# Jan-Celin/SCCG-genome-compression

Measured on AMD Instinct MI355X. Metric: target bases compressed/sec at 1/2/4/8 GPUs; bit-exact record stream vs CPU ref, higher is better.
Workload: dtype u8

## Files before the change

### sccg-genome-compression_amd/csrc/walk.hip

```cpp
#include "internal.h"

#include <algorithm>
#include <chrono>
#include <map>
#include <mutex>
#include <cstdio>
#include <cstdlib>
#include <vector>

namespace {

constexpr int WPB = 4;
constexpr int WWPB = 4;
constexpr int WCAP = 256;
constexpr int32_t INVALID = INT32_MIN;
constexpr int32_t NEVER = INT32_MIN + 1;
constexpr int ANCHOR_K = 32;
constexpr int KEY_K = 15;
constexpr int KMAX = 32;
constexpr int KB_COUNT = 32;
constexpr int ANCHOR_STEP = 64;
constexpr int ANCHOR_LOAD = 1;
constexpr int ANCHOR_PROBE_BATCHES = 2;
constexpr uint32_t A_MULTI = 0xFFFFFFFFu;
// ... 1404 lines not shown
        int32_t e = x0, pe = P0;
        if (i > 0) { e = A.chm_t[i - 1] + A.chm_l[i - 1]; pe = A.chm_p[i - 1] + A.chm_l[i - 1] - 1; }
        sx = e > vc ? e : vc;
        sp = pe;
    };
    int32_t ux, up, i1, ex, ep, i2;
    state_at(lo, lo_c, ux, up, i1);
    state_at(hi, hi_c, ex, ep, i2);
    const int32_t n = i2 - i1;
    const int32_t b = A.cur[q];
    int32_t* ot = A.bt[b] + (size_t)q * A.cap;
    int32_t* op = A.bp[b] + (size_t)q * A.cap;
    int32_t* ol = A.bl[b] + (size_t)q * A.cap;
    for (int32_t i = lane; i < n; i += 64) { ot[i] = A.chm_t[i1 + i]; op[i] = A.chm_p[i1 + i]; ol[i] = A.chm_l[i1 + i]; }
    if (lane == 0) {
        A.cnt[b][q] = n;
        A.usedX[q] = ux; A.usedP[q] = up;
        A.exitX[q] = ex; A.exitP[q] = ep;
        A.changed[q] = 0; A.seedq[q] = 0; A.trapped[q] = 0; A.frozen[q] = 0;
    }
}

__device__ __forceinline__ uint64_t mix64(uint64_t x) {
    x ^= x >> 33; x *= 0xff51afd7ed558ccdull; x ^= x >> 33; x *= 0xc4ceb9fe1a85ec53ull; x ^= x >> 33;
    return x;
}
template <bool ALIGNED>
__device__ __forceinline__ bool code32(const uint8_t* s, uint64_t& code) {
    uint32_t w[8];
    if (ALIGNED) {
        const uint4* p = reinterpret_cast<const uint4*>(s);
        const uint4 a = p[0], b = p[1];
        w[0] = a.x; w[1] = a.y; w[2] = a.z; w[3] = a.w; w[4] = b.x; w[5] = b.y; w[6] = b.z; w[7] = b.w;
    } else {
        loadw<8>(s, w);
    }
    uint32_t bad;
    pack_codes<8>(w, code, bad);
    return bad == 0;
}

constexpr uint32_t ANCHOR_GEN_MASK = 0xfffu;
__device__ __forceinline__ uint64_t anchor_slot(const WalkPtrs& A, uint64_t key, uint32_t pos) {
    return ((uint64_t)(A.agen & ANCHOR_GEN_MASK) << 52) | ((uint64_t)(uint32_t)(key & 0xfffffu) << 32) | pos;
}
__device__ __forceinline__ bool anchor_hit(const WalkPtrs& A, uint64_t key, uint64_t v) {
    return (v >> 32) == (anchor_slot(A, key, 0) >> 32) && (uint32_t)v != A_MULTI;
}
__device__ __forceinline__ void anchor_put(const WalkPtrs& A, uint64_t key, uint32_t pos) {
    if (A.adet) atomicMax((unsigned long long*)&A.atab[key >> (64 - A.abits)], (unsigned long long)anchor_slot(A, key, pos));
    else A.atab[key >> (64 - A.abits)] = anchor_slot(A, key, pos);
}

__device__ __forceinline__ void anchor_samples(const WalkPtrs& A, int64_t nR, int64_t p0, const uint32_t (&cw)[20],
                                               const uint32_t (&dw)[20], uint32_t acc) {
    const int nh = A.astep == 32 ? 2 : 1;
#pragma unroll
    for (int h = 0; h < 2; h++) {
        const int64_t p = p0 + 32 * h;
        if (h >= nh || p + ANCHOR_K > nR) break;
        uint64_t code = 0;
        uint32_t bad = 0;
#pragma unroll
        for (int i = 0; i < 8; i++) {
            code |= (uint64_t)cw[8 * h + i] << (8 * i);
            bad |= dw[8 * h + i];
        }
        if (acc && bad) continue;
        const uint64_t key = mix64(code);
        anchor_put(A, key, (uint32_t)p);
    }
}

__device__ __forceinline__ int32_t anchor_diag_f(int32_t nT, const uint8_t* __restrict__ T, const uint64_t* __restrict__ atab, int32_t abits,
                                 uint32_t agen, int32_t y0) {
    const int lane = lane_id();
    constexpr int NB = ANCHOR_PROBE_BATCHES;
    const uint64_t tag = ((uint64_t)(agen & ANCHOR_GEN_MASK) << 52);
    int32_t dg[NB];
#pragma unroll
    for (int b = 0; b < NB; b++) {
        const int32_t y = y0 + b * 64 + lane;
        dg[b] = INVALID;
        uint64_t code;
        if (y + ANCHOR_K <= nT && code32<false>(T + y, code)) {
            const uint64_t key = mix64(code);
            const uint64_t v = atab[key >> (64 - abits)];
            if ((v >> 32) == ((tag | ((uint64_t)(uint32_t)(key & 0xfffffu) << 32)) >> 32) && (uint32_t)v != A_MULTI)
                dg[b] = (int32_t)(uint32_t)v - y;
        }
    }
    int32_t g = INVALID, first = INVALID;
    int gv = 1;
    for (int tries = 0; tries < 8; tries++) {
        int32_t d = INVALID;
#pragma unroll
        for (int b = 0; b < NB; b++) {
            const unsigned long long m = __ballot(dg[b] != INVALID);
            if (m && d == INVALID) d = __shfl(dg[b], first_lane(m), 64);
        }
        if (d == INVALID) break;
        if (first == INVALID) first = d;
        int votes = 0;
#pragma unroll
        for (int b = 0; b < NB; b++) {
            votes += __popcll(__ballot(dg[b] == d));
            if (dg[b] == d) dg[b] = INVALID;
        }
        if (votes > gv) { g = d; gv = votes; }
    }
    return g == INVALID ? first : g;
}
__device__ int32_t anchor_diag(const WalkPtrs& A, int32_t y0) { return anchor_diag_f(A.nT, A.T, A.atab, A.abits, A.agen, y0); }


constexpr int FC_PER_T = 64;

__device__ __forceinline__ int32_t serial_ext(const uint8_t* R, int32_t nR, const uint8_t* T, int32_t nT, int32_t c,
                                              int32_t y, int k) {
    int32_t l = k;
    while (c + l < nR && y + l < nT && R[c + l] == T[y + l]) ++l;
    return l;
}

template <typename Pred, typename Hit, typename Words>
__device__ __forceinline__ void sweep_kmers_w(const uint8_t* __restrict__ R, int64_t npos, int k, Pred&& pred, Hit&& hit,
                                              Words&& words);
template <typename Pred, typename Hit>
__device__ __forceinline__ void sweep_kmers(const uint8_t* __restrict__ R, int64_t npos, int k, Pred&& pred, Hit&& hit) {
    sweep_kmers_w(R, npos, k, pred, hit, [](int64_t, const uint32_t (&)[20], const uint32_t (&)[20], uint32_t) {});
}
template <typename Pred, typename Hit, typename Words>
__device__ __forceinline__ void sweep_kmers_w(const uint8_t* __restrict__ R, int64_t npos, int k, Pred&& pred, Hit&& hit,
                                              Words&& words) {
    const uint32_t MASK = (1u << (2 * k)) - 1u, KM = (1u << k) - 1u;
    const int64_t stride = (int64_t)gridDim.x * blockDim.x * FC_PER_T;
    for (int64_t p0 = ((int64_t)blockIdx.x * blockDim.x + threadIdx.x) * FC_PER_T; p0 < npos; p0 += stride) {
        uint32_t cw[20], dw[20], acc = 0;
        {
            const uint4* src = reinterpret_cast<const uint4*>(R + p0);
            uint32_t w[20];
#pragma unroll
            for (int i = 0; i < 5; i++) {
                const uint4 v = src[i];
                w[4 * i] = v.x; w[4 * i + 1] = v.y; w[4 * i + 2] = v.z; w[4 * i + 3] = v.w;
            }
#pragma unroll
            for (int i = 0; i < 20; i++) { cw[i] = swar_codes(w[i], dw[i]); acc |= dw[i]; }
        }
        words(p0, cw, dw, acc);
        uint64_t hits = 0;
#pragma unroll
        for (int g = 0; g < 4; g++) {
            uint64_t code = 0;
            uint32_t bad = 0;
#pragma unroll
            for (int i = 0; i < 8; i++) code |= (uint64_t)cw[4 * g + i] << (8 * i);
            if (acc) {
                const uint4* gp = reinterpret_cast<const uint4*>(R + p0 + 16 * g);
                const uint4 v0 = gp[0], v1 = gp[1];
                const uint32_t gw[8] = {v0.x, v0.y, v0.z, v0.w, v1.x, v1.y, v1.z, v1.w};
#pragma unroll
                for (int i = 0; i < 8; i++) { uint32_t d; swar_codes(gw[i], d); bad |= nz_bytes(d) << (4 * i); }
            }
            uint32_t m16 = 0;
            if (!acc) {
#pragma unroll
                for (int st = 15; st >= 0; st--) m16 = (m16 << 1) | (uint32_t)pred((uint32_t)(code >> (2 * st)) & MASK, true);
            } else {
#pragma unroll
                for (int st = 15; st >= 0; st--)
                    m16 = (m16 << 1) | (uint32_t)pred((uint32_t)(code >> (2 * st)) & MASK, ((bad >> st) & KM) == 0);
            }
            hits |= (uint64_t)m16 << (16 * g);
        }
        if (p0 + FC_PER_T > npos) hits &= npos - p0 >= 64 ? ~0ull : ((1ull << (npos - p0)) - 1);
        while (hits) {
            const int b = __ffsll((long long)hits) - 1;
            hits &= hits - 1;
            hit(p0 + b);
        }
    }
}

__global__ void k_fullc(WalkPtrs A, int32_t y, int32_t P, int pass) {
    const int k = A.k, kp = A.kp;
    const uint8_t* kb = A.T + y;
    const uint32_t key = walk_key(kb, kp);
    const uint32_t lmax = (uint32_t)A.fc[0];
    const bool exo = key >= KEY_EXOTIC;
    sweep_kmers(A.R, (int64_t)A.nR - k + 1, kp, [&](uint32_t code, bool pure) {
        return exo ? !pure : (pure && code == key);
    }, [&](int64_t c) {
        if ((exo || k > kp) && !bytes_eq(A.R + c, kb, k)) return;
        const int32_t l = serial_ext(A.R, A.nR, A.T, A.nT, (int32_t)c, y, k);
        if (pass == 0) atomicMax(&A.fc[0], (unsigned long long)l);
        else if ((uint32_t)l == lmax) {
            atomicAdd(&A.fc[1], 1ull);
            if (c == 0) atomicOr(&A.fc[2], 1ull);
            else atomicMin(&A.fc[3], (unsigned long long)pick_key((int32_t)c, P));
        }
    });
}

constexpr int PB = 1024;
constexpr int PBBITS = 11;
constexpr int PRESENCE_GRID = 1024;
constexpr unsigned KEY0_GRID = 1024;
constexpr int KEY0_GRID_MAX = 16384;
constexpr int PFBITS = 17;

struct CandBest {
    uint32_t l, cnt, has0;
    uint64_t minkey;
};
__device__ __forceinline__ CandBest cb_merge(const CandBest& a, const CandBest& b) {
    if (a.l > b.l) return a;
    if (b.l > a.l) return b;
    return CandBest{a.l, a.cnt + b.cnt, a.has0 | b.has0, a.minkey < b.minkey ? a.minkey : b.minkey};
}
__device__ __forceinline__ CandBest cb_shfl_xor(const CandBest& v, int d) {
    return CandBest{(uint32_t)__shfl_xor((int)v.l, d, 64), (uint32_t)__shfl_xor((int)v.cnt, d, 64),
                    (uint32_t)__shfl_xor((int)v.has0, d, 64), (uint64_t)__shfl_xor((unsigned long long)v.minkey, d, 64)};
}
__device__ __forceinline__ CandBest cb_wave(CandBest v) {
#pragma unroll
    for (int d = 32; d > 0; d >>= 1) v = cb_merge(v, cb_shfl_xor(v, d));
    return v;
}

__global__ __launch_bounds__(SCCG_BLOCK) void k_presence(WalkPtrs A, int32_t x0, int32_t nb) {
    __shared__ uint32_t hkey[1 << PBBITS];
    __shared__ uint32_t hidx[1 << PBBITS];
    __shared__ uint32_t bits[1 << (PFBITS - 5)];
    __shared__ CandBest wbest[SCCG_BLOCK / 64];
    const int k = A.k, kp = A.kp;
    const uint32_t key0 = walk_key(A.T + x0, kp);
    CandBest best{0, 0, 0, ~0ull};
    for (int i = threadIdx.x; i < (1 << PBBITS); i += blockDim.x) { hkey[i] = 0xffffffffu; hidx[i] = 0xffffffffu; }
    for (int i = threadIdx.x; i < (1 << (PFBITS - 5)); i += blockDim.x) bits[i] = 0;
    __syncthreads();
    for (int i = threadIdx.x; i < nb; i += blockDim.x) {
        uint32_t w[4], bad;
        uint64_t cw;
        loadw<4>(A.T + x0 + i, w);
        pack_codes<4>(w, cw, bad);
        const uint32_t key = bad & ((1u << kp) - 1u) ? exotic_key(A.T + x0 + i, kp) : (uint32_t)cw & ((1u << (2 * kp)) - 1u);
        if (key >= KEY_EXOTIC) { atomicMin(&A.fc[5], (unsigned long long)(x0 + i)); continue; }
        const uint32_t fb = slot_hash(key, PFBITS);
        atomicOr(&bits[fb >> 5], 1u << (fb & 31));
        int slot = (int)slot_hash(key, PBBITS);
        for (;;) {
            const uint32_t prev = atomicCAS(&hkey[slot], 0xffffffffu, key);
            if (prev == 0xffffffffu || prev == key) { atomicMin(&hidx[slot], (uint32_t)i); break; }
            slot = (slot + 1) & ((1 << PBBITS) - 1);
        }
    }
    __syncthreads();
    sweep_kmers(A.R, (int64_t)A.nR - k + 1, kp, [&](uint32_t code, bool pure) {
        const uint32_t fb = slot_hash(code, PFBITS);
        return pure && ((bits[fb >> 5] >> (fb & 31)) & 1u);
    }, [&](int64_t c) {
        uint64_t cw = 0;
        uint32_t bad;
        uint32_t w[4];
        loadw<4>(A.R + c, w);
        pack_codes<4>(w, cw, bad);
        const uint32_t code = (uint32_t)cw & ((1u << (2 * kp)) - 1u);
        if (code == key0 && (k == kp || bytes_eq(A.R + c + kp, A.T + x0 + kp, k - kp))) {
            const uint32_t l = (uint32_t)serial_ext(A.R, A.nR, A.T, A.nT, (int32_t)c, x0, k);
            best = cb_merge(best, CandBest{l, 1u, c == 0 ? 1u : 0u, c ? pick_key((int32_t)c, -1) : ~0ull});
        }
        int slot = (int)slot_hash(code, PBBITS);
        for (;;) {
            const uint32_t hk = hkey[slot];
            if (hk == 0xffffffffu) break;
            if (hk == code) { atomicMin(&A.fc[4], (unsigned long long)(x0 + hidx[slot])); break; }
            slot = (slot + 1) & ((1 << PBBITS) - 1);
        }
    });
    best = cb_wave(best);
    if (lane_id() == 0) wbest[wave_in_block()] = best;
    __syncthreads();
    if (threadIdx.x == 0) {
        for (int i = 1; i < SCCG_BLOCK / 64; i++) best = cb_merge(best, wbest[i]);
        unsigned long long* o = A.fcb + 4 * blockIdx.x;
        o[0] = best.l; o[1] = best.cnt; o[2] = best.has0; o[3] = best.minkey;
    }
}

template <bool ANCH>
__global__ __launch_bounds__(SCCG_BLOCK) void k_key0(WalkPtrs A, int32_t x0) {
    __shared__ CandBest wbest[SCCG_BLOCK / 64];
    const int k = A.k, kp = A.kp;
    const uint32_t key0 = walk_key(A.T + x0, kp);
    CandBest best{0, 0, 0, ~0ull};
    if (key0 < KEY_EXOTIC || ANCH) {
        const bool want = key0 < KEY_EXOTIC;
        sweep_kmers_w(A.R, (int64_t)A.nR - k + 1, kp, [&](uint32_t code, bool pure) { return want && pure && code == key0; },
                      [&](int64_t c) {
                          if (k > kp && !bytes_eq(A.R + c + kp, A.T + x0 + kp, k - kp)) return;
                          const uint32_t l = (uint32_t)serial_ext(A.R, A.nR, A.T, A.nT, (int32_t)c, x0, k);
                          best = cb_merge(best, CandBest{l, 1u, c == 0 ? 1u : 0u, c ? pick_key((int32_t)c, -1) : ~0ull});
                      },
                      [&](int64_t p0, const uint32_t (&cw)[20], const uint32_t (&dw)[20], uint32_t acc) {
                          if (ANCH) anchor_samples(A, A.nR, p0, cw, dw, acc);
                      });
    }
    best = cb_wave(best);
    if (lane_id() == 0) wbest[wave_in_block()] = best;
    __syncthreads();
    if (threadIdx.x == 0) {
        for (int i = 1; i < SCCG_BLOCK / 64; i++) best = cb_merge(best, wbest[i]);
        unsigned long long* o = A.fcb + 4 * blockIdx.x;
        o[0] = best.l; o[1] = best.cnt; o[2] = best.has0; o[3] = best.minkey;
    }
}

__global__ __launch_bounds__(SCCG_BLOCK) void k_first_kmer(const uint8_t* __restrict__ fa, int64_t n,
                                                           const int64_t* __restrict__ hdr, int k, int64_t limit,
                                                           uint8_t* __restrict__ kb) {
    __shared__ int64_t tmp[5];
    constexpr int PER = 64;
    const int64_t h = hdr[0], he = hdr[1];
    const int64_t end = n < limit ? n : limit;
    int64_t found = 0;
    for (int64_t base = 0; base < end && found < k; base += (int64_t)SCCG_BLOCK * PER) {
        const int64_t p0 = base + (int64_t)threadIdx.x * PER;
        uint32_t w[PER / 4];
        if (p0 + PER + 4 <= end) {
            loadw<PER / 4>(fa + p0, w);
        } else {
#pragma unroll
            for (int q = 0; q < PER / 4; q++) {
                uint32_t v = 0;
                for (int i = 0; i < 4; i++) {
                    const int64_t p = p0 + 4 * q + i;
                    v |= (uint32_t)(p < end ? fa[p] : (uint8_t)' ') << (8 * i);
                }
                w[q] = v;
            }
        }
        uint64_t keep = 0;
#pragma unroll
        for (int i = 0; i < PER; i++) {
            const uint8_t b = (uint8_t)(w[i >> 2] >> (8 * (i & 3)));
            const int64_t p = p0 + i;
            const bool kp = p < end && !(p >= h && p < he) && !c_isspace(b) && c_toupper(b) != 'N';
            keep |= (uint64_t)kp << i;
        }
        int64_t total = 0;
        int64_t idx = found + block_excl_add((int64_t)__popcll(keep), tmp, &total);
        for (uint64_t m = keep; m && idx < k; m &= m - 1, idx++) {
            const int i = __ffsll((long long)m) - 1;
            kb[idx] = c_toupper((uint8_t)(w[i >> 2] >> (8 * (i & 3))));
        }
        found += total;
    }
    if (threadIdx.x == 0) *reinterpret_cast<int32_t*>(kb + KB_COUNT) = found < k ? (int32_t)found : k;
}

__global__ __launch_bounds__(SCCG_BLOCK) void k_sweep_early(WalkPtrs A) {
    const int k = A.k, kp = A.kp;
    const int64_t nR = A.dnR ? *A.dnR : A.nR;
    const bool have = *reinterpret_cast<const int32_t*>(A.kb + KB_COUNT) == k;
    const uint32_t key0 = have ? walk_key(A.kb, kp) : KEY_EXOTIC;
    const bool want = key0 < KEY_EXOTIC;
    sweep_kmers_w(A.R, nR - k + 1, kp, [&](uint32_t code, bool pure) { return want && pure && code == key0; },
                  [&](int64_t c) {
                      if (k > kp && !bytes_eq(A.R + c + kp, A.kb + kp, k - kp)) return;
                      const unsigned long long i = atomicAdd(&A.fc[13], 1ull);
                      if (i < (unsigned long long)CAND_CAP) A.cand[i] = (int32_t)c;
                  },
                  [&](int64_t p0, const uint32_t (&cw)[20], const uint32_t (&dw)[20], uint32_t acc) {
                      anchor_samples(A, nR, p0, cw, dw, acc);
                  });
}

constexpr int CAND_STATS_GRID = 256;
__device__ __forceinline__ bool cand_stats_usable(const WalkPtrs& A) {
    const int k = A.k, lane = lane_id();
    const bool head = *reinterpret_cast<const int32_t*>(A.kb + KB_COUNT) == k && A.fc[13] <= (unsigned long long)CAND_CAP &&
                      A.nT >= k;
    const bool same = lane >= k || A.kb[lane] == A.T[lane];
    return head && __ballot(!same) == 0 && walk_key(A.kb, A.kp) < KEY_EXOTIC;
}
__global__ __launch_bounds__(SCCG_BLOCK) void k_cand_stats(WalkPtrs A) {
    __shared__ CandBest wbest[SCCG_BLOCK / 64];
    __shared__ int ok, last;
    const int k = A.k;
    const unsigned long long cnt = A.fc[13];
    if (threadIdx.x < 64) {
        const bool u = cand_stats_usable(A);
        if (threadIdx.x == 0) ok = u;
    }
    __syncthreads();
    CandBest v{0, 0, 0, ~0ull};
    if (ok) {
        const unsigned long long nw = (unsigned long long)gridDim.x * (SCCG_BLOCK / 64);
        for (unsigned long long i = blockIdx.x * (SCCG_BLOCK / 64) + (threadIdx.x >> 6); i < cnt; i += nw) {
            const int32_t c = A.cand[i];
            int32_t maxlen = A.nR - (c + k);
            if (A.nT - k < maxlen) maxlen = A.nT - k;
            const uint32_t l = (uint32_t)(k + wave_lce_hbm(A.R, c + k, A.T, k, maxlen));
            v = cb_merge(v, CandBest{l, 1u, c == 0 ? 1u : 0u, c ? pick_key(c, -1) : ~0ull});
        }
    }
    if (lane_id() != 0) v = CandBest{0, 0, 0, ~0ull};
    v = cb_wave(v);
    if (lane_id() == 0) wbest[threadIdx.x >> 6] = v;
    __syncthreads();
    if (threadIdx.x == 0) {
        for (int i = 1; i < SCCG_BLOCK / 64; i++) v = cb_merge(v, wbest[i]);
        unsigned long long* o = A.fcb + 4 * blockIdx.x;
        o[0] = v.l; o[1] = v.cnt; o[2] = v.has0; o[3] = v.minkey;
    }
    if (!grid_last_block(reinterpret_cast<unsigned int*>(A.fc + 14), &last)) return;
    if (threadIdx.x == 0) A.fc[12] = ok ? 1 : 2;
    if (!ok) return;
    v = CandBest{0, 0, 0, ~0ull};
    for (int b = (int)threadIdx.x; b < (int)gridDim.x; b += SCCG_BLOCK) {
        const unsigned long long* o = A.fcb + 4 * b;
        v = cb_merge(v, CandBest{(uint32_t)o[0], (uint32_t)o[1], (uint32_t)o[2], o[3]});
    }
    v = cb_wave(v);
    if (lane_id() == 0) wbest[threadIdx.x >> 6] = v;
    __syncthreads();
    if (threadIdx.x == 0) {
// ... 264 lines not shown
        wave_copy(A.T + src, out + dst, len);
    }
}

__global__ __launch_bounds__(SCCG_BLOCK) void k_copy(const uint8_t* __restrict__ in, int64_t n, uint8_t* __restrict__ out) {
    const int64_t G = (int64_t)gridDim.x * WPB;
    for (int64_t o = ((int64_t)blockIdx.x * WPB + wave_in_block()) * LONG_PIECE; o < n; o += G * LONG_PIECE)
        wave_copy(in + o, out + o, n - o < LONG_PIECE ? n - o : LONG_PIECE);
}

struct Carve {
    char* base;
    size_t off, cap;
    template <typename T>
    T* take(size_t n) {
        off = (off + 255) & ~(size_t)255;
        T* p = reinterpret_cast<T*>(base + off);
        off += n * sizeof(T);
        return p;
    }
};

int env_int(const char* name, int dflt) {
    const char* e = getenv(name);
    return e ? atoi(e) : dflt;
}
struct WalkEnv {
    bool debug;
    bool phases;
    int debug_round;
    int debug_rounds;
    bool all_rounds;
    int debug_chunk;
    int round_log;
};
const WalkEnv& walk_env() {
    static const WalkEnv e = [] {
        const char* rl = getenv("SCCG_ROUND_LOG");
        return WalkEnv{getenv("SCCG_DEBUG") != nullptr,       getenv("SCCG_DEBUG_PHASES") != nullptr,
                       env_int("SCCG_DEBUG_ROUND", -1),       env_int("SCCG_DEBUG_ROUNDS", 3),
                       getenv("SCCG_DEBUG_ALLROUNDS") != nullptr, env_int("SCCG_DEBUG_CHUNK", -1),
                       rl ? (rl[0] == '2' ? 2 : 1) : 0};
    }();
    return e;
}

int anchor_bits(int64_t nR) {
    static const int shift = [] { const int x = env_int("SCCG_ANCHOR_SHIFT", 0); return x >= -4 && x <= 4 ? x : 0; }();
    int64_t want = ANCHOR_LOAD * (nR / ANCHOR_STEP + 1);
    int b = 10;
    while ((1ll << b) < want && b < 34) b++;
    b += shift;
    return b < 10 ? 10 : b;
}

WalkPtrs carve(void* ws, size_t ws_bytes, const uint8_t* R, int64_t nR, const uint8_t* T, int64_t nT, int k, int m,
               int S, size_t* used, int abits = 0) {
    WalkPtrs A{};
    Carve c{(char*)ws, 0, ws_bytes};
    A.R = R; A.T = T;
    A.nR = (int32_t)nR; A.nT = (int32_t)nT; A.k = k; A.m = m; A.S = S;
    A.kp = k < KEY_K ? k : KEY_K;
    A.C = (int32_t)((nT + S - 1) / S);
    if (A.C < 1) A.C = 1;
    A.xlo = 0;
    A.xhi = (int32_t)nT;
    A.cap = S / k + 4;
    const size_t C = (size_t)A.C, cap = (size_t)A.cap;
    A.abits = abits ? abits : anchor_bits(nR);
    A.astep = ANCHOR_STEP;
    A.atab = c.take<uint64_t>((size_t)1 << A.abits);
    A.fc = c.take<unsigned long long>(16);
    A.fcb = c.take<unsigned long long>(4 * KEY0_GRID_MAX);
    A.cand = c.take<int32_t>(CAND_CAP);
    A.kb = c.take<uint8_t>(64);
    for (int b = 0; b < 2; b++) {
        A.bt[b] = c.take<int32_t>(C * cap);
        A.bp[b] = c.take<int32_t>(C * cap);
        A.bl[b] = c.take<int32_t>(C * cap);
        A.cnt[b] = c.take<int32_t>(C);
    }
    A.cur = c.take<int32_t>(C);
    A.exitX = c.take<int32_t>(C); A.exitP = c.take<int32_t>(C);
    A.usedX = c.take<int32_t>(C); A.usedP = c.take<int32_t>(C);
    A.kind = c.take<int32_t>(C); A.status = c.take<int32_t>(C);
    A.escX = c.take<int32_t>(C); A.escP = c.take<int32_t>(C); A.escN = c.take<int32_t>(C); A.escQ = c.take<int32_t>(C);
    A.snapX = c.take<int32_t>(C); A.snapP = c.take<int32_t>(C);
    A.guess = c.take<int32_t>(C);
    A.plist = c.take<int32_t>(C);
    A.rlist = c.take<int32_t>(C);
    A.clist = c.take<int32_t>(C);
    A.newX = c.take<int32_t>(C); A.newP = c.take<int32_t>(C);
    A.conv = c.take<int32_t>(C); A.changed = c.take<int32_t>(C); A.walked = c.take<int32_t>(C);
    A.lround = c.take<int32_t>(C);
    A.seedq = c.take<int32_t>(C);
    A.trapped = c.take<int32_t>(C);
    A.frozen = c.take<int32_t>(C); A.flist = c.take<int32_t>(C);
    A.fbits = c.take<uint32_t>(C / 32 + 1); A.cbits = c.take<uint32_t>(C / 32 + 1);
    A.fy = c.take<int32_t>(FROZEN_MAX);
    A.scal = c.take<int32_t>(16);
    A.trig = c.take<int32_t>(RESPEC_MAX_TRIGGERS);
    A.tflag = c.take<int32_t>(C);
    A.fa_j = c.take<int32_t>(FROZEN_MAX); A.fa_l = c.take<int32_t>(FROZEN_MAX); A.fa_p = c.take<int32_t>(FROZEN_MAX);
    A.hintY = c.take<int32_t>(C); A.hintP = c.take<int32_t>(C);
    A.flat_off = c.take<int64_t>(C + 1);
    const size_t maxm = (size_t)(nT / k + 2);
    A.ft = c.take<int32_t>(maxm); A.fp = c.take<int32_t>(maxm); A.fl = c.take<int32_t>(maxm);
    A.tlen = c.take<int64_t>(maxm + 1);
    A.partial = c.take<int64_t>((size_t)scan_partials_needed((int64_t)(maxm > C ? maxm : C) + 1) + 16);
    A.scal64 = c.take<int64_t>(8);
    A.lgap_cap = nT / LONG_GAP + nT / LONG_PIECE + 2;
    A.lgap = c.take<int64_t>(3 * (size_t)A.lgap_cap);
    A.cprev = c.take<int64_t>(C + 1);
    A.ctext = c.take<int64_t>(C + 1);
    A.chs = c.take<int32_t>(16);
    {
        const int64_t mc = nT / k + 2;
        const int64_t lim = CH_HANDBACK_N + 1 < CHAIN_MCAP ? CH_HANDBACK_N + 1 : CHAIN_MCAP;
        A.chm_cap = (int32_t)(mc < lim ? mc : lim);
    }
    A.chm_t = c.take<int32_t>((size_t)A.chm_cap);
    A.chm_p = c.take<int32_t>((size_t)A.chm_cap);
    A.chm_l = c.take<int32_t>((size_t)A.chm_cap);
    A.chh_y = c.take<int32_t>((size_t)CH_GRID * CH_HCAP);
    A.chh_k = c.take<uint32_t>((size_t)CH_GRID * CH_HCAP);
    A.chh_n = c.take<int32_t>(CH_GRID);
    A.chh_tr = c.take<int32_t>(CH_GRID);
    A.dbg = c.take<uint64_t>(C * DBG_SLOTS);
    *used = c.off;
    return A;
}

using WalkKernel = void (*)(WalkPtrs, const int32_t*, int32_t, const int32_t*);
WalkKernel walk_kernel(const WalkPtrs& A) { return A.dbg ? k_walk<true, false> : k_walk<false, false>; }
constexpr int CARRY_GRID = 256;
int launch_carry(const WalkPtrs& A, hipStream_t s) {
    hipLaunchKernelGGL(k_list_sort, dim3(1), dim3(LS_T), 0, s, A, A.clist, (const int32_t*)(A.scal + 11), A.cbits);
    PROF_LAUNCH(PROF_WALK_CARRY, s, (A.dbg ? k_walk<true, true> : k_walk<false, true>), dim3(CARRY_GRID), dim3(64 * WWPB), 0, s, A,
                (const int32_t*)A.clist, 0, (const int32_t*)(A.scal + 11));
    SCCG_HIP(hipGetLastError());
    return 0;
}

struct FullC {
    int64_t lmax;
    int32_t p;
};

int set_u64(unsigned long long* p, std::initializer_list<int64_t> v, hipStream_t s) {
    return dev_set_i64(reinterpret_cast<int64_t*>(p), (int)v.size(), v, s);
}

int run_fullc(WalkPtrs& A, int32_t y, int32_t P, FullC* out, hipStream_t s) {
    int rc = set_u64(A.fc, {0, 0, 0, -1}, s);
    if (rc) return rc;
    const int64_t npos = (int64_t)A.nR - A.k + 1;
    unsigned g = grid_for(npos > 0 ? npos : 1, 256 * FC_PER_T);
    if (g > 8192) g = 8192;
    PROF_LAUNCH(PROF_FULLC, s, k_fullc, dim3(g), dim3(256), 0, s, A, y, P, 0);
    PROF_LAUNCH(PROF_FULLC, s, k_fullc, dim3(g), dim3(256), 0, s, A, y, P, 1);
    SCCG_HIP(hipGetLastError());
    unsigned long long r[4];
    {
        const RbItem it{A.fc, r, (int)sizeof r};
        const int rc = dev_readback(&it, 1, s);
        if (rc) return rc;
    }
    out->lmax = (int64_t)r[0];
    if (r[0] == 0) { out->p = INVALID; return 0; }
    const uint64_t k0 = (uint64_t)(uint32_t)(P < 0 ? -P : P) << 32;
    uint64_t pk;
    if (r[1] >= 2 && r[2]) pk = r[3];
    else pk = (r[2] && k0 < r[3]) ? k0 : r[3];
    out->p = (int32_t)(uint32_t)pk;
    return 0;
}

int h2d_sync(void* dst, const void* src, size_t bytes, hipStream_t s) {
    if (!bytes) return 0;
    SCCG_HIP(hipMemcpyAsync(dst, src, bytes, hipMemcpyHostToDevice, s));
    SCCG_HIP(hipStreamSynchronize(s));
    return 0;
}

int run_chain(WalkPtrs& A, hipStream_t s, int* gens, bool* trapped, bool* started) {
    hipLaunchKernelGGL(k_chain_init, dim3(1), dim3(64), 0, s, A);
    SCCG_HIP(hipGetLastError());
    int32_t st[5] = {0, 0, 0, 0, 0};
    *started = true;
    for (int it = 0;; it++) {
        for (int g = 0; g < CH_GENS_PER_SYNC; g++) {
            hipLaunchKernelGGL(k_chain_scan, dim3(CH_GRID), dim3(1024), 0, s, A);
            hipLaunchKernelGGL(k_chain_step, dim3(1), dim3(64), 0, s, A);
        }
        SCCG_HIP(hipGetLastError());
        const RbItem it0{A.chs, st, (int)sizeof st};
        const int rc = dev_readback(&it0, 1, s);
        if (rc) return rc;
        if (!st[0] && st[4] < 0) {
            *started = false;
            *gens = 0;
            *trapped = false;
            return 0;
        }
        if (!st[0]) break;
        if (it > CH_MAX_GENS / CH_GENS_PER_SYNC + 1) return SCCG_E_INTERNAL;
    }
    PROF_LAUNCH(PROF_WALK_CHAIN, s, k_chain_fill, dim3(grid_for(A.C, WPB)), dim3(SCCG_BLOCK), 0, s, A);
    SCCG_HIP(hipGetLastError());
    int32_t cs[12];
    {
// ... 46 lines not shown
        if (rc) return rc;
        if ((rc = h2d_sync(A.rlist, rl.data(), rl.size() * 4, s))) return rc;
        PROF_LAUNCH(PROF_WALK, s, walk_kernel(A), dim3(grid_for((int64_t)rl.size(), WWPB)), dim3(64 * WWPB), 0, s, A,
                    (const int32_t*)A.rlist, (int32_t)rl.size(), (const int32_t*)nullptr);
        SCCG_HIP(hipGetLastError());
    }
}

}

size_t walk_workspace_bytes(int64_t nR, int64_t nT, int k, int chunk) {
    size_t used = 0;
    carve(nullptr, 0, nullptr, nR, nullptr, nT, k, 100, chunk, &used);
    return used + 4096;
}

static thread_local WalkPtrs g_last;
static thread_local int64_t g_last_n = 0;

int global_matches(void* , const int32_t** t, const int32_t** p, const int32_t** l, int64_t* n) {
    *t = g_last.ft; *p = g_last.fp; *l = g_last.fl; *n = g_last_n;
    return 0;
}

#define RC(expr)                      \
    do {                              \
        int rc_ = (expr);             \
        if (rc_) return rc_;          \
    } while (0)

namespace {

struct Prepared {
    const void* ws = nullptr;
    const uint8_t* R = nullptr;
    const uint8_t* T = nullptr;
    int64_t nR = -1, nT = -1;
    int k = 0, m = 0, chunk = 0;
    uint32_t agen = 0;
    int abits = 0;
};
thread_local Prepared g_prep;

struct Early {
    const void* ws = nullptr;
    const uint8_t* R = nullptr;
    int64_t nR = -1;
    int k = 0;
    uint32_t agen = 0;
    int abits = 0;
};
thread_local Early g_early;

unsigned first_sweep_grid(const WalkPtrs& A) {
    const unsigned g = grid_for(A.nR - A.k + 1, 256 * FC_PER_T);
    return g > KEY0_GRID ? KEY0_GRID : g;
}

struct AnchorSeen { const uint64_t* tab; size_t clean; uint32_t gen; };
std::mutex g_anchor_mu;
std::map<const void*, AnchorSeen> g_anchor_seen;

int anchor_generation(WalkPtrs& A, const void* ws, hipStream_t s) {
    const size_t n = (size_t)1 << A.abits;
    uint32_t g;
    bool clear;
    {
        std::lock_guard<std::mutex> lk(g_anchor_mu);
        AnchorSeen& e = g_anchor_seen[ws];
        clear = e.tab != A.atab || n > e.clean || e.gen >= ANCHOR_GEN_MASK;
        if (clear) e.gen = 0;
        e.tab = A.atab;
        e.clean = n;
        g = ++e.gen;
    }
    if (clear) SCCG_HIP(hipMemsetAsync(A.atab, 0, n * sizeof(uint64_t), s));
    A.agen = g;
    return 0;
}

int queue_prepare(WalkPtrs& A, const void* ws, hipStream_t s) {
    const int32_t lastk = A.nT - A.k;
    const bool walkable = A.nR >= A.k && lastk >= 0;
    if (!walkable) return 0;
    const unsigned gsweep = first_sweep_grid(A);
    RC(anchor_generation(A, ws, s));
    PROF_LAUNCH(PROF_ANCHOR, s, k_key0<true>, dim3(gsweep), dim3(SCCG_BLOCK), 0, s, A, 0);
    hipLaunchKernelGGL(k_cand_reduce, dim3(1), dim3(1024), 0, s, A, (int)gsweep, 0);
    SCCG_HIP(hipGetLastError());
    return 0;
}

WalkPtrs make_ptrs(const uint8_t* Rp, int64_t nRp, const uint8_t* Tp, int64_t nTp, int k, int m, int chunk, void* ws,
                   size_t ws_bytes, size_t* used, int abits = 0) {
    WalkPtrs A = carve(ws, ws_bytes, Rp, nRp, Tp, nTp, k, m, chunk, used, abits);
    if (!walk_env().debug) A.dbg = nullptr;
    A.dbg_phases = walk_env().phases;
    A.dbg_round = walk_env().debug_round;
    A.adet = env_int("SCCG_ANCHOR_DET", 0);
    return A;
}

}

void global_prepare_reset() { g_prep = Prepared{}; g_early = Early{}; }

int global_sweep_early(const uint8_t* Rp, int64_t nRp, const int64_t* d_nRp, const uint8_t* tgt_fa, int64_t tn,
                       const int64_t* d_hdr, int k, int m, int chunk, void* ws, size_t ws_bytes, hipStream_t s_head,
                       hipEvent_t ev_head, hipStream_t s) {
    g_early = Early{};
    if (m < 0 || 2 * m + 1 > WCAP || k > KMAX || k < 1) return SCCG_E_UNSUPPORTED;
    if (nRp < k || tn <= 0) return 0;
    size_t used = 0;
    WalkPtrs A = make_ptrs(Rp, nRp, nullptr, tn, k, m, chunk, ws, ws_bytes, &used);
    if (used > ws_bytes) return SCCG_E_INTERNAL;
    A.dnR = d_nRp;
    RC(anchor_generation(A, ws, s_head));
    RC(set_u64(A.fc + 12, {0, 0, 0}, s_head));
    hipLaunchKernelGGL(k_first_kmer, dim3(1), dim3(SCCG_BLOCK), 0, s_head, tgt_fa, tn, d_hdr, k, (int64_t)1 << 20, A.kb);
    SCCG_HIP(hipEventRecord(ev_head, s_head));
    SCCG_HIP(hipStreamWaitEvent(s, ev_head, 0));
    PROF_LAUNCH(PROF_ANCHOR, s, k_sweep_early, dim3(first_sweep_grid(A)), dim3(SCCG_BLOCK), 0, s, A);
    SCCG_HIP(hipGetLastError());
    g_early = Early{ws, Rp, nRp, k, A.agen, A.abits};
    return 0;
}

int global_prepare(const uint8_t* Rp, int64_t nRp, const uint8_t* Tp, int64_t nTp, int k, int m, int chunk, void* ws,
                   size_t ws_bytes, hipStream_t s) {
    g_prep = Prepared{};
    if (m < 0 || 2 * m + 1 > WCAP || k > KMAX || k < 1) return SCCG_E_UNSUPPORTED;
    const Early e = g_early;
    g_early = Early{};
    const bool early = e.ws == ws && e.R == Rp && e.nR >= nRp && e.k == k;
    size_t used = 0;
    WalkPtrs A = make_ptrs(Rp, nRp, Tp, nTp, k, m, chunk, ws, ws_bytes, &used, early ? e.abits : 0);
    if (used > ws_bytes) return SCCG_E_INTERNAL;
    if (early) {
        A.agen = e.agen;
        if (A.nR >= A.k && A.nT >= A.k) {
            hipLaunchKernelGGL(k_cand_stats, dim3(CAND_STATS_GRID), dim3(SCCG_BLOCK), 0, s, A);
            SCCG_HIP(hipGetLastError());
        }
    } else {
        RC(queue_prepare(A, ws, s));
    }
    g_prep = Prepared{ws, Rp, Tp, nRp, nTp, k, m, chunk, A.agen, A.abits};
    return 0;
}

namespace {
struct RangeWalk {
    int64_t x0 = 0, P0 = -1, x_end = 0;
    int64_t exit_x = 0, exit_P = -1;
};

struct WalkRun {
    WalkPtrs A;
    hipStream_t s;
    WalkResult* res;
    const EmitTarget* late_out;
    RangeWalk* rw;
    uint8_t* out;
    bool abs_p, keep_flat;
    const uint8_t* Tp;
    int64_t nTp;
    int32_t lastk;
    int32_t first_y = INVALID, first_p = 0, first_l = 0;
    int32_t startX = 0, startP = INVALID;
    bool pre_round = false;
    bool spec_queued = false;
    bool spec_text = false;
    bool text_done = false;
    bool resolved = false;
    int32_t rs_pre[6] = {};
// ... 38 lines not shown
    SCCG_HIP(hipGetLastError());
    RC(launch_round_end(A, 0, fbase_cap, s));
    return 0;
}

int WalkRun::queue_text(bool long_copy, bool dev_first) {
    const int32_t nf = dev_first ? 2 : first_y != INVALID ? 1 : 0;
    if (A.C <= CP_MAX) {
        hipLaunchKernelGGL(k_chunk_prefix, dim3(1), dim3(1024), 0, s, A);
    } else {
        const unsigned gc = grid_for(A.C, 256) > 4096 ? 4096 : grid_for(A.C, 256);
        hipLaunchKernelGGL(k_chunk_meta, dim3(gc), dim3(256), 0, s, A);
        RC(dev_excl_max(A.cprev, A.cprev, A.C, nullptr, A.partial, s));
        RC(dev_excl_sum(A.flat_off, A.flat_off, A.C, A.scal64, A.partial, s));
        RC(set_u64(reinterpret_cast<unsigned long long*>(A.scal64 + 2), {0}, s));
    }
    const FirstMatch F{first_y, first_p, first_l, nf};
    hipLaunchKernelGGL(k_chunk_text<false>, dim3(grid_for(A.C, WPB)), dim3(SCCG_BLOCK), 0, s, A, F, (int)abs_p, out);
    RC(dev_excl_sum(A.ctext, A.ctext, A.C, A.scal64 + 1, A.partial, s));
    PROF_LAUNCH(PROF_MATCH_EMIT, s, k_chunk_text<true>, dim3(grid_for(A.C, WPB)), dim3(SCCG_BLOCK), 0, s, A, F,
                (int)abs_p, out);
    if (long_copy) hipLaunchKernelGGL(k_long_copy, dim3(1024), dim3(256), 0, s, A, out);
    SCCG_HIP(hipGetLastError());
    return 0;
}

int WalkRun::frozen_batch(int fbase, int fcap, bool init_fy) {
    if (init_fy) SCCG_HIP(hipMemsetD32Async((hipDeviceptr_t)A.fy, INT32_MAX, fcap, s));
    if (fcap > 0) hipLaunchKernelGGL(k_frozen_scan, dim3(FZ_GRID, fcap), dim3(FZ_T), 0, s, A, fbase);
    SCCG_HIP(hipGetLastError());
    RC(launch_round_end(A, fbase, fcap, s));
    return 0;
}

int WalkRun::first_step() {
    const int k = A.k;
    int32_t x0 = 0;
    unsigned long long r[9];
    if (pre_round) {
        if (!keep_flat && !walk_env().debug) {
            RC(resolve_out());
            RC(queue_text(true, true));
            spec_queued = true;
        }
        const RbItem it[3] = {{A.fc + 4, r, (int)sizeof r}, {A.scal, rs_pre, (int)sizeof rs_pre},
                              {A.scal64, spec_r, (int)sizeof spec_r}};
        RC(dev_readback(it, 3, s));
        if (!(r[8] != 2 && r[0] == 0 && r[4] > 0)) { pre_round = false; spec_queued = false; }
    } else {
        const RbItem it{A.fc + 4, r, (int)sizeof r};
        RC(dev_readback(&it, 1, s));
    }
    if (r[8] == 2) {
        const unsigned g = first_sweep_grid(A);
        hipLaunchKernelGGL(k_key0<false>, dim3(g), dim3(SCCG_BLOCK), 0, s, A, 0);
        hipLaunchKernelGGL(k_cand_reduce, dim3(1), dim3(1024), 0, s, A, (int)g, 0);
        SCCG_HIP(hipGetLastError());
        const RbItem it{A.fc + 4, r, (int)sizeof r};
        RC(dev_readback(&it, 1, s));
    }
    if (r[0] == 0 && r[4] > 0) {
        first_y = 0;
        const uint64_t k0 = 1ull << 32;
        const uint64_t pk = (r[5] >= 2 && r[6]) ? r[7] : ((r[6] && k0 < r[7]) ? k0 : r[7]);
        first_p = (int32_t)(uint32_t)pk;
        first_l = (int32_t)r[4];
    }
    const int64_t npos = (int64_t)A.nR - k + 1 > 0 ? (int64_t)A.nR - k + 1 : 1;
    const unsigned gsweep = grid_for(npos, 256 * FC_PER_T) > PRESENCE_GRID ? PRESENCE_GRID : grid_for(npos, 256 * FC_PER_T);
    while (x0 <= lastk && first_y == INVALID) {
        const int32_t nb = (lastk - x0 + 1) < PB ? (lastk - x0 + 1) : PB;
        RC(set_u64(A.fc + 4, {-1, -1}, s));
        PROF_LAUNCH(PROF_PRESENCE, s, k_presence, dim3(gsweep), dim3(SCCG_BLOCK), 0, s, A, x0, nb);
        hipLaunchKernelGGL(k_cand_reduce, dim3(1), dim3(1024), 0, s, A, (int)gsweep, -1);
        SCCG_HIP(hipGetLastError());
        {
            const RbItem it{A.fc + 4, r, (int)sizeof r};
            RC(dev_readback(&it, 1, s));
        }
        if (r[0] != ~0ull && r[0] < r[1]) {
            const int32_t y = (int32_t)r[0];
            if (y == x0 && r[4] > 0) {
                const uint64_t k0 = 1ull << 32;
                const uint64_t pk = (r[5] >= 2 && r[6]) ? r[7] : ((r[6] && k0 < r[7]) ? k0 : r[7]);
                first_y = y;
                first_p = (int32_t)(uint32_t)pk;
                first_l = (int32_t)r[4];
                break;
            }
            if (A.k == A.kp) { first_y = y; break; }
            FullC f;
            RC(run_fullc(A, y, -1, &f, s));
            if (f.lmax > 0) { first_y = y; first_p = f.p; first_l = (int32_t)f.lmax; break; }
            x0 = y + 1;
            continue;
        }
        if (r[1] != ~0ull) {
            FullC f;
            RC(run_fullc(A, (int32_t)r[1], -1, &f, s));
            if (f.lmax > 0) { first_y = (int32_t)r[1]; break; }
            x0 = (int32_t)r[1] + 1;
            continue;
        }
        x0 += nb;
    }
    if (first_y != INVALID && first_l == 0) {
        FullC f;
        RC(run_fullc(A, first_y, -1, &f, s));
        first_p = f.p;
        first_l = (int32_t)f.lmax;
    }
    return 0;
}

int WalkRun::probe_frozen_first(bool* frozen_first) {
    RC(dev_set_i32(A.flist, 1, {0}, s));
    RC(dev_set_i32(A.exitX, 1, {startX}, s));
    RC(dev_set_i32(A.exitP, 1, {startP}, s));
    RC(dev_set_i32(A.scal + 5, 1, {1}, s));
    RC(dev_set_i32(A.fy, 1, {INT32_MAX}, s));
    hipLaunchKernelGGL(k_frozen_scan, dim3(FZ_GRID, 1), dim3(FZ_T), 0, s, A, 0);
    SCCG_HIP(hipGetLastError());
// ... 450 lines not shown
```

Before: 188.7 billion.

## Restructure k-mer sweep to wave-coalesced tiles with prefetch and key filter

Rewrites the reference k-mer sweep so each wave processes a contiguous span with lane-interleaved 16-byte loads. Neighbour codes come from cross-lane shuffles instead of per-thread 80-byte reloads, and the next tile is software-prefetched. Adds a SWAR prefilter for single-key sweeps that skips per-position predicate evaluation when no match is possible, and a cold path for tiles containing non-ACGT bytes. Grid sizes now derive from occupancy queries instead of fixed caps. This risks more shuffle overhead and register pressure, and adds complexity in the handling of bad bytes at tile boundaries.

```diff
diff --git a/sccg-genome-compression_amd/csrc/walk.hip b/sccg-genome-compression_amd/csrc/walk.hip
--- a/sccg-genome-compression_amd/csrc/walk.hip
+++ b/sccg-genome-compression_amd/csrc/walk.hip
@@ -1480,24 +1480,11 @@
     else A.atab[key >> (64 - A.abits)] = anchor_slot(A, key, pos);
 }
 
-__device__ __forceinline__ void anchor_samples(const WalkPtrs& A, int64_t nR, int64_t p0, const uint32_t (&cw)[20],
-                                               const uint32_t (&dw)[20], uint32_t acc) {
-    const int nh = A.astep == 32 ? 2 : 1;
-#pragma unroll
-    for (int h = 0; h < 2; h++) {
-        const int64_t p = p0 + 32 * h;
-        if (h >= nh || p + ANCHOR_K > nR) break;
-        uint64_t code = 0;
-        uint32_t bad = 0;
-#pragma unroll
-        for (int i = 0; i < 8; i++) {
-            code |= (uint64_t)cw[8 * h + i] << (8 * i);
-            bad |= dw[8 * h + i];
-        }
-        if (acc && bad) continue;
-        const uint64_t key = mix64(code);
-        anchor_put(A, key, (uint32_t)p);
-    }
+__device__ __forceinline__ void anchor_sample(const WalkPtrs& A, int64_t nR, int64_t q, uint32_t mine, uint32_t next,
+                                              uint32_t bad) {
+    if ((q & (int64_t)(A.astep - 1)) != 0 || q + ANCHOR_K > nR || bad) return;
+    const uint64_t key = mix64((uint64_t)mine | ((uint64_t)next << 32));
+    anchor_put(A, key, (uint32_t)q);
 }
 
 __device__ __forceinline__ int32_t anchor_diag_f(int32_t nT, const uint8_t* __restrict__ T, const uint64_t* __restrict__ atab, int32_t abits,
@@ -1542,8 +1529,6 @@
 __device__ int32_t anchor_diag(const WalkPtrs& A, int32_t y0) { return anchor_diag_f(A.nT, A.T, A.atab, A.abits, A.agen, y0); }
 
 
-constexpr int FC_PER_T = 64;
-
 __device__ __forceinline__ int32_t serial_ext(const uint8_t* R, int32_t nR, const uint8_t* T, int32_t nT, int32_t c,
                                               int32_t y, int k) {
     int32_t l = k;
@@ -1551,64 +1536,137 @@
     return l;
 }
 
-template <typename Pred, typename Hit, typename Words>
-__device__ __forceinline__ void sweep_kmers_w(const uint8_t* __restrict__ R, int64_t npos, int k, Pred&& pred, Hit&& hit,
-                                              Words&& words);
-template <typename Pred, typename Hit>
-__device__ __forceinline__ void sweep_kmers(const uint8_t* __restrict__ R, int64_t npos, int k, Pred&& pred, Hit&& hit) {
-    sweep_kmers_w(R, npos, k, pred, hit, [](int64_t, const uint32_t (&)[20], const uint32_t (&)[20], uint32_t) {});
-}
-template <typename Pred, typename Hit, typename Words>
-__device__ __forceinline__ void sweep_kmers_w(const uint8_t* __restrict__ R, int64_t npos, int k, Pred&& pred, Hit&& hit,
-                                              Words&& words) {
+constexpr int SW_PIECES = 4;
+constexpr int SW_SPAN = 64 * 16 * SW_PIECES;
+constexpr int SW_BLOCK_SPAN = (SCCG_BLOCK / 64) * SW_SPAN;
+static_assert(ANCHOR_STEP == 64 && SW_SPAN == 64 * ANCHOR_STEP, "a wave iteration holds one sample per lane");
+
+__device__ __forceinline__ uint32_t sweep_pack(const uint4& v, uint32_t& flag) {
+    const uint32_t xl = __builtin_amdgcn_perm(v.y, v.x, 0x05010400u), xh = __builtin_amdgcn_perm(v.y, v.x, 0x07030602u);
+    const uint32_t zl = __builtin_amdgcn_perm(v.w, v.z, 0x05010400u), zh = __builtin_amdgcn_perm(v.w, v.z, 0x07030602u);
+    const uint32_t u[4] = {__builtin_amdgcn_perm(zl, xl, 0x05040100u), __builtin_amdgcn_perm(zl, xl, 0x07060302u),
+                           __builtin_amdgcn_perm(zh, xh, 0x05040100u), __builtin_amdgcn_perm(zh, xh, 0x07060302u)};
+    uint32_t c[4];
+    flag = 0;
+#pragma unroll
+    for (int i = 0; i < 4; i++) {
+        c[i] = ((u[i] >> 1) ^ (u[i] >> 2)) & 0x03030303u;
+        flag |= __builtin_amdgcn_perm(0x54474341u, 0x54474341u, c[i]) ^ u[i];
+    }
+    return c[0] | (c[1] << 2) | (c[2] << 4) | (c[3] << 6);
+}
+__device__ __forceinline__ uint32_t sweep_bad(const uint4& v) {
+    uint32_t d0, d1, d2, d3;
+    (void)swar_codes(v.x, d0); (void)swar_codes(v.y, d1); (void)swar_codes(v.z, d2); (void)swar_codes(v.w, d3);
+    return nz_bytes(d0) | (nz_bytes(d1) << 4) | (nz_bytes(d2) << 8) | (nz_bytes(d3) << 12);
+}
+
+__device__ __forceinline__ void sweep_load(const uint8_t* __restrict__ R, int64_t nR, int64_t b0, int lane, uint4 (&v)[SW_PIECES + 1]) {
+#pragma unroll
+    for (int j = 0; j <= SW_PIECES; j++) {
+        const int64_t q = b0 + 1024 * j + (j < SW_PIECES ? 16 * lane : 0);
+        v[j] = *reinterpret_cast<const uint4*>(R + (q < nR ? q : 0));
+    }
+}
+
+constexpr int SW_FILTER = 8;
+template <bool SINGLE, typename Pred, typename Hit, typename Words>
+__device__ __forceinline__ void sweep_kmers_w(const uint8_t* __restrict__ R, int64_t nR, int64_t npos, int k, uint32_t key,
+                                              Pred&& pred, Hit&& hit, Words&& words) {
     const uint32_t MASK = (1u << (2 * k)) - 1u, KM = (1u << k) - 1u;
-    const int64_t stride = (int64_t)gridDim.x * blockDim.x * FC_PER_T;
-    for (int64_t p0 = ((int64_t)blockIdx.x * blockDim.x + threadIdx.x) * FC_PER_T; p0 < npos; p0 += stride) {
-        uint32_t cw[20], dw[20], acc = 0;
-        {
-            const uint4* src = reinterpret_cast<const uint4*>(R + p0);
-            uint32_t w[20];
+    const int lane = lane_id();
+    uint32_t kb[SW_FILTER];
 #pragma unroll
-            for (int i = 0; i < 5; i++) {
-                const uint4 v = src[i];
-                w[4 * i] = v.x; w[4 * i + 1] = v.y; w[4 * i + 2] = v.z; w[4 * i + 3] = v.w;
+    for (int i = 0; i < SW_FILTER; i++) kb[i] = 0x55555555u * ((key >> (2 * i)) & 3u);
+    const bool filter = SINGLE && k >= SW_FILTER;
+    const int64_t stride = (int64_t)gridDim.x * (blockDim.x >> 6) * SW_SPAN;
+    int64_t b0 = ((int64_t)blockIdx.x * (blockDim.x >> 6) + wave_in_block()) * SW_SPAN;
+    uint4 v[SW_PIECES + 1];
+    if (b0 < npos) sweep_load(R, nR, b0, lane, v);
+    for (; b0 < npos; b0 += stride) {
+        uint32_t cw[SW_PIECES + 1], bd[SW_PIECES + 1], anybad = 0;
+#pragma unroll
+        for (int j = 0; j <= SW_PIECES; j++) {
+            const int64_t q = b0 + 1024 * j + (j < SW_PIECES ? 16 * lane : 0);
+            uint32_t flag;
+            cw[j] = sweep_pack(v[j], flag);
+            anybad |= q < nR ? flag : 1u;
+            bd[j] = 0;
+        }
+        const bool wbad = __ballot(anybad != 0) != 0;
+        if (!wbad) {
+            const int src = 4 * (lane & 15);
+            uint32_t lo = 0, hi = 0;
+#pragma unroll
+            for (int j = 0; j < SW_PIECES; j++) {
+                const uint32_t a = (uint32_t)__shfl((int)cw[j], src, 64), b = (uint32_t)__shfl((int)cw[j], src + 1, 64);
+                if ((lane >> 4) == j) { lo = a; hi = b; }
             }
+            words(b0 + 64 * lane, lo, hi, 0u);
+        }
+        __builtin_amdgcn_sched_barrier(0);
+        if (b0 + stride < npos) sweep_load(R, nR, b0 + stride, lane, v);
+        __builtin_amdgcn_sched_barrier(0);
+        if (wbad) {
+#pragma unroll 1
+            for (int j = 0; j <= SW_PIECES; j++) {
+                const int64_t q = b0 + 1024 * j + (j < SW_PIECES ? 16 * lane : 0);
+                const uint32_t m = q < nR ? sweep_bad(*reinterpret_cast<const uint4*>(R + q)) : 0xffffu;
 #pragma unroll
-            for (int i = 0; i < 20; i++) { cw[i] = swar_codes(w[i], dw[i]); acc |= dw[i]; }
-        }
-        words(p0, cw, dw, acc);
+                for (int i = 0; i <= SW_PIECES; i++) bd[i] = i == j ? m : bd[i];
+            }
+        }
         uint64_t hits = 0;
 #pragma unroll
-        for (int g = 0; g < 4; g++) {
-            uint64_t code = 0;
+        for (int j = 0; j < SW_PIECES; j++) {
+            const int64_t q = b0 + 1024 * j + 16 * lane;
+            const uint32_t mine = cw[j];
+            const uint32_t row_c = lane_val(cw[j + 1], 0);
+            const uint32_t dn_c = (uint32_t)__shfl_down((int)mine, 1, 64);
+            const uint32_t next = lane == 63 ? row_c : dn_c;
             uint32_t bad = 0;
-#pragma unroll
-            for (int i = 0; i < 8; i++) code |= (uint64_t)cw[4 * g + i] << (8 * i);
-            if (acc) {
-                const uint4* gp = reinterpret_cast<const uint4*>(R + p0 + 16 * g);
-                const uint4 v0 = gp[0], v1 = gp[1];
-                const uint32_t gw[8] = {v0.x, v0.y, v0.z, v0.w, v1.x, v1.y, v1.z, v1.w};
-#pragma unroll
-                for (int i = 0; i < 8; i++) { uint32_t d; swar_codes(gw[i], d); bad |= nz_bytes(d) << (4 * i); }
+            if (wbad) {
+                const uint32_t row_b = lane_val(bd[j + 1], 0);
+                const uint32_t dn_b = (uint32_t)__shfl_down((int)bd[j], 1, 64);
+                bad = bd[j] | ((lane == 63 ? row_b : dn_b) << 16);
+                words(q, mine, next, bad);
             }
             uint32_t m16 = 0;
-            if (!acc) {
+            if (bad == 0) {
+                bool any = false;
+                if (filter) {
+                    uint32_t acc = mine ^ kb[0];
 #pragma unroll
-                for (int st = 15; st >= 0; st--) m16 = (m16 << 1) | (uint32_t)pred((uint32_t)(code >> (2 * st)) & MASK, true);
+                    for (int i = 1; i < SW_FILTER; i++) acc |= __builtin_amdgcn_alignbit(next, mine, 2 * i) ^ kb[i];
+                    any = ((acc | (acc >> 1)) & 0x55555555u) != 0x55555555u;
+                } else {
+#pragma unroll
+                    for (int st = 0; st < 16; st++) any |= pred(__builtin_amdgcn_alignbit(next, mine, 2 * st) & MASK, true);
+                }
+                if (any) {
+#pragma unroll 1
+                    for (int st = 0; st < 16; st++)
+                        m16 |= (uint32_t)pred(__builtin_amdgcn_alignbit(next, mine, 2 * st) & MASK, true) << st;
+                }
             } else {
-#pragma unroll
-                for (int st = 15; st >= 0; st--)
-                    m16 = (m16 << 1) | (uint32_t)pred((uint32_t)(code >> (2 * st)) & MASK, ((bad >> st) & KM) == 0);
+#pragma unroll 1
+                for (int st = 0; st < 16; st++)
+                    m16 |= (uint32_t)pred(__builtin_amdgcn_alignbit(next, mine, 2 * st) & MASK, ((bad >> st) & KM) == 0) << st;
             }
-            hits |= (uint64_t)m16 << (16 * g);
-        }
-        if (p0 + FC_PER_T > npos) hits &= npos - p0 >= 64 ? ~0ull : ((1ull << (npos - p0)) - 1);
+            if (q + 16 > npos) m16 &= q >= npos ? 0u : (1u << (int)(npos - q)) - 1u;
+            hits |= (uint64_t)m16 << (16 * j);
+        }
         while (hits) {
             const int b = __ffsll((long long)hits) - 1;
             hits &= hits - 1;
-            hit(p0 + b);
-        }
-    }
+            hit(b0 + 1024 * (b >> 4) + 16 * lane + (b & 15));
+        }
+    }
+}
+template <typename Pred, typename Hit>
+__device__ __forceinline__ void sweep_kmers(const uint8_t* __restrict__ R, int64_t nR, int64_t npos, int k, Pred&& pred,
+                                            Hit&& hit) {
+    sweep_kmers_w<false>(R, nR, npos, k, 0u, pred, hit, [](int64_t, uint32_t, uint32_t, uint32_t) {});
 }
 
 __global__ void k_fullc(WalkPtrs A, int32_t y, int32_t P, int pass) {
@@ -1617,7 +1675,7 @@
     const uint32_t key = walk_key(kb, kp);
     const uint32_t lmax = (uint32_t)A.fc[0];
     const bool exo = key >= KEY_EXOTIC;
-    sweep_kmers(A.R, (int64_t)A.nR - k + 1, kp, [&](uint32_t code, bool pure) {
+    sweep_kmers(A.R, (int64_t)A.nR, (int64_t)A.nR - k + 1, kp, [&](uint32_t code, bool pure) {
         return exo ? !pure : (pure && code == key);
     }, [&](int64_t c) {
         if ((exo || k > kp) && !bytes_eq(A.R + c, kb, k)) return;
@@ -1634,7 +1692,7 @@
 constexpr int PB = 1024;
 constexpr int PBBITS = 11;
 constexpr int PRESENCE_GRID = 1024;
-constexpr unsigned KEY0_GRID = 1024;
+constexpr unsigned KEY0_GRID = 1536;
 constexpr int KEY0_GRID_MAX = 16384;
 constexpr int PFBITS = 17;
 
@@ -1685,7 +1743,7 @@
         }
     }
     __syncthreads();
-    sweep_kmers(A.R, (int64_t)A.nR - k + 1, kp, [&](uint32_t code, bool pure) {
+    sweep_kmers(A.R, (int64_t)A.nR, (int64_t)A.nR - k + 1, kp, [&](uint32_t code, bool pure) {
         const uint32_t fb = slot_hash(code, PFBITS);
         return pure && ((bits[fb >> 5] >> (fb & 31)) & 1u);
     }, [&](int64_t c) {
@@ -1724,15 +1782,14 @@
     const uint32_t key0 = walk_key(A.T + x0, kp);
     CandBest best{0, 0, 0, ~0ull};
     if (key0 < KEY_EXOTIC || ANCH) {
-        const bool want = key0 < KEY_EXOTIC;
-        sweep_kmers_w(A.R, (int64_t)A.nR - k + 1, kp, [&](uint32_t code, bool pure) { return want && pure && code == key0; },
+        sweep_kmers_w<true>(A.R, (int64_t)A.nR, (int64_t)A.nR - k + 1, kp, uni(key0), [&](uint32_t code, bool pure) { return pure && code == key0; },
                       [&](int64_t c) {
                           if (k > kp && !bytes_eq(A.R + c + kp, A.T + x0 + kp, k - kp)) return;
                           const uint32_t l = (uint32_t)serial_ext(A.R, A.nR, A.T, A.nT, (int32_t)c, x0, k);
                           best = cb_merge(best, CandBest{l, 1u, c == 0 ? 1u : 0u, c ? pick_key((int32_t)c, -1) : ~0ull});
                       },
-                      [&](int64_t p0, const uint32_t (&cw)[20], const uint32_t (&dw)[20], uint32_t acc) {
-                          if (ANCH) anchor_samples(A, A.nR, p0, cw, dw, acc);
+                      [&](int64_t q, uint32_t mine, uint32_t next, uint32_t bad) {
+                          if (ANCH) anchor_sample(A, A.nR, q, mine, next, bad);
                       });
     }
     best = cb_wave(best);
@@ -1793,15 +1850,14 @@
     const int64_t nR = A.dnR ? *A.dnR : A.nR;
     const bool have = *reinterpret_cast<const int32_t*>(A.kb + KB_COUNT) == k;
     const uint32_t key0 = have ? walk_key(A.kb, kp) : KEY_EXOTIC;
-    const bool want = key0 < KEY_EXOTIC;
-    sweep_kmers_w(A.R, nR - k + 1, kp, [&](uint32_t code, bool pure) { return want && pure && code == key0; },
+    sweep_kmers_w<true>(A.R, nR, nR - k + 1, kp, uni(key0), [&](uint32_t code, bool pure) { return pure && code == key0; },
                   [&](int64_t c) {
                       if (k > kp && !bytes_eq(A.R + c + kp, A.kb + kp, k - kp)) return;
                       const unsigned long long i = atomicAdd(&A.fc[13], 1ull);
                       if (i < (unsigned long long)CAND_CAP) A.cand[i] = (int32_t)c;
                   },
-                  [&](int64_t p0, const uint32_t (&cw)[20], const uint32_t (&dw)[20], uint32_t acc) {
-                      anchor_samples(A, nR, p0, cw, dw, acc);
+                  [&](int64_t q, uint32_t mine, uint32_t next, uint32_t bad) {
+                      anchor_sample(A, nR, q, mine, next, bad);
                   });
 }
 
@@ -2172,6 +2228,13 @@
     while ((1ll << b) < want && b < 34) b++;
     b += shift;
     return b < 10 ? 10 : b;
+}
+
+unsigned sweep_grid(int64_t npos, unsigned cap) {
+    static const int env_cap = [] { const int x = env_int("SCCG_SWEEP_GRID", 0); return x >= 1 && x <= KEY0_GRID_MAX ? x : 0; }();
+    if (env_cap && (unsigned)env_cap < cap) cap = (unsigned)env_cap;
+    const unsigned g = grid_for(npos > 0 ? npos : 1, SW_BLOCK_SPAN);
+    return g > cap ? cap : g;
 }
 
 WalkPtrs carve(void* ws, size_t ws_bytes, const uint8_t* R, int64_t nR, const uint8_t* T, int64_t nT, int k, int m,
@@ -2275,8 +2338,7 @@
     int rc = set_u64(A.fc, {0, 0, 0, -1}, s);
     if (rc) return rc;
     const int64_t npos = (int64_t)A.nR - A.k + 1;
-    unsigned g = grid_for(npos > 0 ? npos : 1, 256 * FC_PER_T);
-    if (g > 8192) g = 8192;
+    const unsigned g = sweep_grid(npos, 8192);
     PROF_LAUNCH(PROF_FULLC, s, k_fullc, dim3(g), dim3(256), 0, s, A, y, P, 0);
     PROF_LAUNCH(PROF_FULLC, s, k_fullc, dim3(g), dim3(256), 0, s, A, y, P, 1);
     SCCG_HIP(hipGetLastError());
@@ -2429,9 +2491,28 @@
 };
 thread_local Early g_early;
 
-unsigned first_sweep_grid(const WalkPtrs& A) {
-    const unsigned g = grid_for(A.nR - A.k + 1, 256 * FC_PER_T);
-    return g > KEY0_GRID ? KEY0_GRID : g;
+unsigned resident_blocks(const void* kernel) {
+    static std::mutex mu;
+    static std::map<std::pair<int, const void*>, unsigned> seen;
+    int dev = 0;
+    if (hipGetDevice(&dev) != hipSuccess) return KEY0_GRID;
+    std::lock_guard<std::mutex> lk(mu);
+    auto it = seen.find({dev, kernel});
+    if (it != seen.end()) return it->second;
+    int per_cu = 0, cus = 0;
+    unsigned g = KEY0_GRID;
+    if (hipOccupancyMaxActiveBlocksPerMultiprocessor(&per_cu, kernel, SCCG_BLOCK, 0) == hipSuccess &&
+        hipDeviceGetAttribute(&cus, hipDeviceAttributeMultiprocessorCount, dev) == hipSuccess && per_cu > 0 && cus > 0)
+        g = (unsigned)per_cu * (unsigned)cus;
+    else
+        (void)hipGetLastError();
+    if (g > (unsigned)KEY0_GRID_MAX) g = KEY0_GRID_MAX;
+    seen[{dev, kernel}] = g;
+    return g;
+}
+template <typename K>
+unsigned first_sweep_grid(const WalkPtrs& A, K kernel) {
+    return sweep_grid((int64_t)A.nR - A.k + 1, resident_blocks(reinterpret_cast<const void*>(kernel)));
 }
 
 struct AnchorSeen { const uint64_t* tab; size_t clean; uint32_t gen; };
@@ -2460,7 +2541,7 @@
     const int32_t lastk = A.nT - A.k;
     const bool walkable = A.nR >= A.k && lastk >= 0;
     if (!walkable) return 0;
-    const unsigned gsweep = first_sweep_grid(A);
+    const unsigned gsweep = first_sweep_grid(A, k_key0<true>);
     RC(anchor_generation(A, ws, s));
     PROF_LAUNCH(PROF_ANCHOR, s, k_key0<true>, dim3(gsweep), dim3(SCCG_BLOCK), 0, s, A, 0);
     hipLaunchKernelGGL(k_cand_reduce, dim3(1), dim3(1024), 0, s, A, (int)gsweep, 0);
@@ -2497,7 +2578,7 @@
     hipLaunchKernelGGL(k_first_kmer, dim3(1), dim3(SCCG_BLOCK), 0, s_head, tgt_fa, tn, d_hdr, k, (int64_t)1 << 20, A.kb);
     SCCG_HIP(hipEventRecord(ev_head, s_head));
     SCCG_HIP(hipStreamWaitEvent(s, ev_head, 0));
-    PROF_LAUNCH(PROF_ANCHOR, s, k_sweep_early, dim3(first_sweep_grid(A)), dim3(SCCG_BLOCK), 0, s, A);
+    PROF_LAUNCH(PROF_ANCHOR, s, k_sweep_early, dim3(first_sweep_grid(A, k_sweep_early)), dim3(SCCG_BLOCK), 0, s, A);
     SCCG_HIP(hipGetLastError());
     g_early = Early{ws, Rp, nRp, k, A.agen, A.abits};
     return 0;
@@ -2642,7 +2723,7 @@
         RC(dev_readback(&it, 1, s));
     }
     if (r[8] == 2) {
-        const unsigned g = first_sweep_grid(A);
+        const unsigned g = first_sweep_grid(A, k_key0<false>);
         hipLaunchKernelGGL(k_key0<false>, dim3(g), dim3(SCCG_BLOCK), 0, s, A, 0);
         hipLaunchKernelGGL(k_cand_reduce, dim3(1), dim3(1024), 0, s, A, (int)g, 0);
         SCCG_HIP(hipGetLastError());
@@ -2657,7 +2738,7 @@
         first_l = (int32_t)r[4];
     }
     const int64_t npos = (int64_t)A.nR - k + 1 > 0 ? (int64_t)A.nR - k + 1 : 1;
-    const unsigned gsweep = grid_for(npos, 256 * FC_PER_T) > PRESENCE_GRID ? PRESENCE_GRID : grid_for(npos, 256 * FC_PER_T);
+    const unsigned gsweep = sweep_grid(npos, PRESENCE_GRID);
     while (x0 <= lastk && first_y == INVALID) {
         const int32_t nb = (lastk - x0 + 1) < PB ? (lastk - x0 + 1) : PB;
         RC(set_u64(A.fc + 4, {-1, -1}, s));
```

Result: no change. 187.6 billion, median of 2 (-0.6%).
